# AiRyunn/BoT

Hardware: AMD Instinct MI355X
Metric: edges/sec full-batch GAT fwd+bwd on ogbn-arxiv; achieved HBM GB/s vs peak (higher is better)
Workload: dtype f32

## Files before the change

bot_amd/_C.py:

```python
from __future__ import annotations

import ctypes
import os
from ctypes import c_char_p, c_double, c_float, c_int32, c_int64, c_uint64, c_void_p

import torch

_HERE = os.path.dirname(os.path.abspath(__file__))
LIB_PATH = os.environ.get("BOT_AMD_LIB") or os.path.join(_HERE, "lib", "libbot_gnn.so")
ABI_VERSION = 19

if not os.path.exists(LIB_PATH):
    raise ImportError(
        f"{LIB_PATH} is missing: build the gfx950 kernels first "
        "(`make -C bot_amd/csrc` or `python -c 'import __graft_entry__ as g; g.build()'`). "
        "bot_amd has no CPU / PyTorch fallback."
    )
_lib = ctypes.CDLL(LIB_PATH)

_P = c_void_p
_SIGS = {
    "bot_abi_version": (ctypes.c_int, []),
    "bot_last_error": (c_char_p, []),
    "bot_last_kernel": (c_char_p, []),
# ... 897 lines not shown
    def fits(self, m, n, k) -> bool:
        return (m == self.n and n == self.F and self.F % 2 == 0 and self.x.stride(0) % 2 == 0 and self.x.data_ptr() % 8 == 0 and
                _lib.bot_gemm_halves3_nt_bn_rows(int(k)) == 256)

    def struct(self):
        return _BnBwdStats(self.x.data_ptr(), self.x.stride(0), self.mean.data_ptr(), self.invstd.data_ptr(), _ptr(self.weight), _ptr(self.bias),
                           int(self.relu), self.p, self.seed, _seed_off(self.p), self.part.data_ptr(), _ptr(self.pmax))

    def sums(self):
        sg = torch.empty(self.F, dtype=torch.float32, device=self.x.device)
        sgx = torch.empty(self.F, dtype=torch.float32, device=self.x.device)
        _check(_lib.bot_bn_act_bwd_reduce_partials_f32(self.part.data_ptr(), self.nblk, self.F, sg.data_ptr(), sgx.data_ptr(), _stream()),
               "bn_act_bwd_reduce_partials")
        return sg, sgx

    def finish(self, batch_stats, total_count, slots):
        assert self.pmax is not None
        _dev(slots)
        sg = torch.empty(self.F, dtype=torch.float32, device=self.x.device)
        sgx = torch.empty(self.F, dtype=torch.float32, device=self.x.device)
        _check(_lib.bot_bn_bwd_partials_finish_f32(self.part.data_ptr(), self.pmax.data_ptr(), self.nblk, self.F, sg.data_ptr(), sgx.data_ptr(),
                                                   int(bool(batch_stats)), float(total_count), _ptr(self.weight), self.invstd.data_ptr(), slots.data_ptr(),
                                                   _stream()), "bn_bwd_partials_finish")
        return sg, sgx

    def bound(self, sum_g, sum_gx, total_count, slots):
        assert self.pmax is not None
        _dev(slots)
        _check(_lib.bot_bn_bwd_bound_partials_f32(self.F, self.pmax.data_ptr(), self.nblk, _ptr(sum_g), _ptr(sum_gx), float(total_count), _ptr(self.weight),
                                                  self.invstd.data_ptr(), slots.data_ptr(), _stream()), "bn_bwd_bound_partials")
        return slots


def gemm_halves3_nt(a, b, scale_a, scale_b, piece_a, piece_b, k, out=None, mode=0, a2_off=None, scale_a2=None, k_split=0, b_frag=False, n=None, bn=None):
    _dev(a, b, scale_a, scale_b, scale_a2)
    m = a.shape[0]
    if n is None:
        assert not b_frag
        n = b.shape[0]
    if out is None:
        out = torch.empty((m, n), dtype=torch.float32, device=a.device)
    st = None
    if bn is not None:
        if not bn.fits(m, n, k):
            raise BotKernelError("gemm_halves3_nt: this product cannot carry the BatchNorm-backward by-product (BnBwdStats.fits)")
        st = bn.struct()
    _check(_timed("gemm_halves", (m, n, 3 * k, 1), lambda: _lib.bot_gemm_halves3_nt3_f32(
        m, n, k, scale_a.data_ptr(), _ptr(scale_a2), int(k_split), scale_b.data_ptr(), a.data_ptr(), _ld(a), 2 * piece_a if a2_off is None else a2_off,
        b.data_ptr(), _ld(b), piece_b, int(bool(b_frag)), out.data_ptr(), _ld(out), ctypes.addressof(st) if st is not None else None, int(mode), _stream())),
        "gemm_halves3_nt")
    return out


def halves_split_frag(x, scale, piece):
    _dev(x, scale)
    x = _mat(x, "x")
    n, F = x.shape
    assert piece % 64 == 0 and piece >= F
    out = torch.empty((2 * ((n + 15) // 16) * (piece // 32), 512), dtype=torch.float16, device=x.device)
    _check(_lib.bot_halves_split_frag_f16(x.data_ptr(), x.stride(0), n, F, _ptr(scale), out.data_ptr(), piece, _stream()), "halves_split_frag")
    return out


def _table(rows, width):
    flat = [int(v) for r in rows for v in r]
    assert len(flat) == width * len(rows)
    return (ctypes.c_int64 * len(flat))(*flat)


def gemm_halves3_nt_grouped(a, b, scale_a, scale_b, a2_off, b2_off, out, groups, k_seg, mode=0, col_scale=None, col_shift=None, relu=False, absmax=None,
                            stats=None):
    _dev(a, b, out, scale_a, scale_b, col_scale, col_shift, absmax)
    assert a.dtype == torch.float16 and b.dtype == torch.float16 and a.dim() == 2 and b.dim() == 2 and a.stride(1) == 1 and b.stride(1) == 1
    assert out.dtype == torch.float32 and out.stride(-1) == 1
    tab = _table(groups, 6)
    sp = sm = sv = None
    sF = 0
    if stats is not None:
        sp, sm, sv = stats
        _dev(sp, sm, sv)
        sF = sv.shape[1]
        tiles = (a.shape[0] + 255) // 256
        assert sp.shape == (tiles, 2, sF) and sm.shape == (tiles, 2, sF) and sv.shape == (tiles, sF)
        assert sp.is_contiguous() and sm.is_contiguous() and sv.is_contiguous()
        assert sp.dtype == sm.dtype == sv.dtype == torch.float32
    _check(_timed("gemm_halves", (a.shape[0], sum(int(g[1]) * 96 * int(g[4]) for g in groups), 1, 1), lambda: _lib.bot_gemm_halves3_nt_grouped2_f32(
        a.shape[0], b.shape[0], scale_a.data_ptr(), scale_b.data_ptr(), a.data_ptr(), _ld(a), a2_off, b.data_ptr(), _ld(b), b2_off, out.data_ptr(),
        int(out.stride(-2)), len(groups), tab, int(k_seg), _ptr(col_scale), _ptr(col_shift), int(bool(relu)), _ptr(absmax), _ptr(sp), _ptr(sm), _ptr(sv),
        int(sF), int(mode), _stream())), "gemm_halves3_nt_grouped")
    return out


def gemm_halves3_tn_grouped(x, d, scale_x, scale_d, x2_off, d2_off, out, tiles, mode=0):
    _dev(x, d, out, scale_x, scale_d)
    assert x.dtype == torch.float16 and d.dtype == torch.float16 and x.stride(1) == 1 and d.stride(1) == 1 and x.shape[0] == d.shape[0]
    assert out.dtype == torch.float32 and out.is_contiguous()
    n = x.shape[0]
    ws = torch.empty(int(_lib.bot_gemm_halves3_tn_grouped_workspace_floats(n, len(tiles))), dtype=torch.float32, device=x.device)
    tab = _table(tiles, 7)
    _check(_timed("gemm_halves", (n, sum(3 * int(t[1]) * int(t[3]) for t in tiles), 1, 1), lambda: _lib.bot_gemm_halves3_tn_grouped_f32(
        n, scale_x.data_ptr(), scale_d.data_ptr(), x.data_ptr(), _ld(x), x2_off, d.data_ptr(), _ld(d), d2_off, out.data_ptr(), len(tiles), tab,
        ws.data_ptr(), int(mode), _stream())), "gemm_halves3_tn_grouped")
    return out


def gemm_halves3_tn(x, d, scale_x, scale_d, piece_x, piece_d, k, p, mode=0, x2_off=None, d2_off=None, scale_d2=None, p_split=0):
    _dev(x, d, scale_x, scale_d, scale_d2)
    n = x.shape[0]
    out = torch.empty((k, p), dtype=torch.float32, device=x.device)
    ws = torch.empty(int(_lib.bot_gemm_halves3_tn_workspace_floats(n, piece_x, piece_d)), dtype=torch.float32, device=x.device)
    _check(_timed("gemm_halves", (k, p, 3 * n, 1), lambda: _lib.bot_gemm_halves3_tn2_f32(
        n, k, p, piece_x, piece_d, scale_x.data_ptr(), scale_d.data_ptr(), _ptr(scale_d2), int(p_split), x.data_ptr(), _ld(x),
        2 * piece_x if x2_off is None else x2_off, d.data_ptr(), _ld(d), 2 * piece_d if d2_off is None else d2_off,
        out.data_ptr(), _ld(out), ws.data_ptr(), int(mode), _stream())), "gemm_halves3_tn")
    return out


def _idx64(t, name):
    if t.dtype != torch.int64 or not t.is_contiguous() or t.dim() != 1:
        raise BotKernelError(f"{name} must be a contiguous 1-D int64 tensor (got {t.dtype}, stride {tuple(t.stride())})")


# ... 568 lines not shown
```

bot_amd/csrc/halves3.hip:

```cpp
#include <hip/hip_fp16.h>

#include <stdlib.h>
#include <string.h>

#include <algorithm>
#include <type_traits>
#include <utility>

#include "common.h"

namespace bot {
namespace {

constexpr int BK = 32;

typedef _Float16 half8 __attribute__((ext_vector_type(8)));
typedef float f32x4 __attribute__((ext_vector_type(4)));

struct H3Args {
    const _Float16* A;
    const _Float16* B;
    const float* scale_a;
    const float* scale_b;
    float* C;
// ... 652 lines not shown
    if constexpr (BNB) {
#pragma unroll
        for (int e = 0; e < 4; ++e) {
#pragma unroll
            for (int o = 8; o < 64; o <<= 1) {
                b_s[e] += __shfl_xor(b_s[e], o);
                b_q[e] += __shfl_xor(b_q[e], o);
                b_gm[e] = fmaxf(b_gm[e], __shfl_xor(b_gm[e], o));
                b_xm[e] = fmaxf(b_xm[e], __shfl_xor(b_xm[e], o));
            }
        }
        if (lane < 8) {
            const int64_t F = p.N;
            float* ps = p.bnb_part + ((int64_t)tm * 2) * F + c0 + col;
#pragma unroll
            for (int e = 0; e < 4; ++e)
                if (e < b_nv) ps[e] = b_s[e], ps[F + e] = b_q[e];
            if (p.bnb_pmax) {
                float* pm = p.bnb_pmax + ((int64_t)tm * 2) * F + c0 + col;
#pragma unroll
                for (int e = 0; e < 4; ++e)
                    if (e < b_nv) pm[e] = b_gm[e], pm[F + e] = b_xm[e];
            }
        }
    }
}

__global__ __launch_bounds__(512) void gemm_halves3_nt64_kernel(H3Args p) { gemm_halves3_nt64_body<false, false>(p, nullptr); }
__global__ __launch_bounds__(512) void gemm_halves3_nt64_frag_kernel(H3Args p) { gemm_halves3_nt64_body<false, true>(p, nullptr); }
__global__ __launch_bounds__(512) void gemm_halves3_nt64_grouped_kernel(H3Args p, H3Groups groups) { gemm_halves3_nt64_body<true, false>(p, &groups); }
__global__ __launch_bounds__(512) void gemm_halves3_nt64_bnb_kernel(H3Args p) { gemm_halves3_nt64_body<false, false, true>(p, nullptr); }
__global__ __launch_bounds__(512) void gemm_halves3_nt64_frag_bnb_kernel(H3Args p) { gemm_halves3_nt64_body<false, true, true>(p, nullptr); }

static bool nt64_wanted() {
    static const bool wanted = [] {
        const char* e = getenv("BOT_NT_KERNEL");
        return !(e && !strcmp(e, "128x64"));
    }();
    return wanted;
}

constexpr int TBK = 32;
constexpr int TT = 192;
constexpr int kTnSubA = TBK * 256, kTnSubB = TBK * 128;
constexpr int kTnPiece = kTnSubA + kTnSubB;
constexpr int kTnStage = 4 * kTnPiece;
constexpr int kTnStages = 3;

struct TnArgs3 {
    const _Float16* X;
    const _Float16* D;
    float* part;
    int64_t ldx, ldd;
    int N, K, P, KP, PP;
    int x2_off, d2_off;
    int tiles_k, tiles_p, splits, rows_per_split;
    int mode;
};


struct TnTile {
    int x_col0, d_col0, k_valid, p_valid;
    int64_t out_off, ldo;
    int transposed, pad;
};
constexpr int kMaxTnTiles = 16;
// ... 273 lines not shown
}

template <int BM, int BN, int WM, int WN, bool PIPE, bool ABLATE>
void launch_h3(H3Args p, int64_t m, int64_t n, hipStream_t st) {
    p.tiles_m = (int)((m + BM - 1) / BM), p.tiles_n = (int)((n + BN - 1) / BN);
    const int groups = (p.tiles_m + 7) / 8;
    hipLaunchKernelGGL((gemm_halves3_nt_kernel<BM, BN, WM, WN, PIPE, ABLATE>), dim3(groups * 8 * p.tiles_n), dim3(WM * WN * 64), 0, st, p);
}

}
}

extern "C" int bot_gemm_halves3_nt_f32(int64_t m, int64_t n, int64_t k, const float* scale_a, const float* scale_b, const uint16_t* A, int64_t lda,
                                       int64_t a2_off, const uint16_t* B, int64_t ldb, int64_t b2_off, float* C, int64_t ldc, int32_t mode,
                                       bot_stream_t stream) {
    return bot_gemm_halves3_nt2_f32(m, n, k, scale_a, nullptr, 0, scale_b, A, lda, a2_off, B, ldb, b2_off, 0, C, ldc, mode, stream);
}

extern "C" int bot_gemm_halves3_nt2_f32(int64_t m, int64_t n, int64_t k, const float* scale_a, const float* scale_a2, int64_t k_split, const float* scale_b,
                                        const uint16_t* A, int64_t lda, int64_t a2_off, const uint16_t* B, int64_t ldb, int64_t b2_off, int32_t b_layout,
                                        float* C, int64_t ldc, int32_t mode, bot_stream_t stream) {
    return bot_gemm_halves3_nt3_f32(m, n, k, scale_a, scale_a2, k_split, scale_b, A, lda, a2_off, B, ldb, b2_off, b_layout, C, ldc, nullptr, mode, stream);
}

extern "C" int32_t bot_gemm_halves3_nt_bn_rows(int64_t k) {
    using namespace bot;
    return (k > 0 && k % (2 * BK) == 0 && nt64_wanted()) ? 256 : 0;
}

extern "C" int bot_gemm_halves3_nt3_f32(int64_t m, int64_t n, int64_t k, const float* scale_a, const float* scale_a2, int64_t k_split, const float* scale_b,
                                        const uint16_t* A, int64_t lda, int64_t a2_off, const uint16_t* B, int64_t ldb, int64_t b2_off, int32_t b_layout,
                                        float* C, int64_t ldc, const bot_bn_bwd_stats_t* bn, int32_t mode, bot_stream_t stream) {
    using namespace bot;
    BOT_REQUIRE(bn == nullptr || (mode == 0 && bot_gemm_halves3_nt_bn_rows(k) == 256), -1,
                "gemm_halves3_nt3: the BatchNorm-backward by-product rides on the 256 x 32 form (mode 0, k a multiple of 64, BOT_NT_KERNEL not 128x64)");
    BOT_REQUIRE(bn == nullptr || (bn->x && bn->mean && bn->invstd && bn->part), -1, "gemm_halves3_nt3: bn->x, mean, invstd and part must be set");
    BOT_REQUIRE(bn == nullptr || (n % 2 == 0 && bn->ldx >= n && bn->ldx % 2 == 0 && aligned(bn->x, 8) && bn->p >= 0.f && bn->p < 1.f), -1,
                "gemm_halves3_nt3: the by-product needs an even n (= the BatchNorm width), 8-byte aligned x rows of pitch >= n and p in [0, 1)");
    BOT_REQUIRE(b_layout == 0 || (b_layout == 1 && mode == 0 && k % 64 == 0), -1,
                "gemm_halves3_nt2: b_layout 1 (fragment-major B, bot_halves_split_frag_f16 with piece = k) needs mode 0 and k a multiple of 64");
    BOT_REQUIRE(scale_a2 == nullptr || (k_split > 0 && k_split < k && k_split % BK == 0), -1,
                "gemm_halves3_nt2: the second scale starts at a column that is a positive multiple of %d below k (got %lld of %lld)", BK, (long long)k_split,
                (long long)k);
    BOT_REQUIRE(m > 0 && n > 0 && k > 0 && k % BK == 0, -1, "gemm_halves3_nt: m, n > 0 and k a positive multiple of %d (got %lld %lld %lld)", BK,
                (long long)m, (long long)n, (long long)k);
    BOT_REQUIRE(scale_a && scale_b && A && B && C, -1, "gemm_halves3_nt: null pointer");
    BOT_REQUIRE(aligned(A, 16) && aligned(B, 16) && lda % 8 == 0 && ldb % 8 == 0 && a2_off % 8 == 0 && b2_off % 8 == 0, -1,
                "gemm_halves3_nt: operands, row pitches and piece offsets must be 16-byte aligned");
    BOT_REQUIRE(a2_off + k <= lda && (b_layout == 1 || b2_off + k <= ldb) && ldc >= n && m < (1ll << 31) - 256 && n < (1ll << 31) - 256, -1, "gemm_halves3_nt: bad pitches");
    BOT_REQUIRE(b_layout == 0 || ((n + 15) / 16) * (k / 32) * 2048 < (1ll << 31), -1, "gemm_halves3_nt2: fragment-major B exceeds the 2 GiB a buffer descriptor spans");
    H3Args p;
    p.A = reinterpret_cast<const _Float16*>(A), p.B = reinterpret_cast<const _Float16*>(B), p.scale_a = scale_a, p.scale_b = scale_b, p.C = C;
    p.lda = lda, p.ldb = ldb, p.ldc = ldc, p.M = (int)m, p.N = (int)n, p.K = (int)k, p.a2_off = (int)a2_off, p.b2_off = (int)b2_off;
    p.tiles_m = p.tiles_n = 0;
    p.col_scale = p.col_shift = nullptr, p.relu = 0, p.absmax = nullptr;
    p.scale_a2 = scale_a2, p.k2 = scale_a2 ? (int)(k_split / BK) : -1;
    p.b_frag = b_layout;
    p.stats_part = p.stats_minmax = nullptr, p.stats_pivot = nullptr, p.stats_F = 0;
    p.bnb_x = nullptr, p.bnb_ldx = 0, p.bnb_mean = p.bnb_invstd = p.bnb_w = p.bnb_b = nullptr, p.bnb_relu = 0, p.bnb_p = 0.f, p.bnb_seed = 0;
    p.bnb_seed_offset = nullptr, p.bnb_part = p.bnb_pmax = nullptr;
    p.mode = mode;
    const bool force_128x64 = (mode & 1024) != 0;
    mode &= ~1024;
    p.mode = mode;
    if (bn) {
        p.bnb_x = bn->x, p.bnb_ldx = bn->ldx, p.bnb_mean = bn->mean, p.bnb_invstd = bn->invstd, p.bnb_w = bn->weight, p.bnb_b = bn->bias;
        p.bnb_relu = bn->relu, p.bnb_p = bn->p, p.bnb_seed = bn->seed, p.bnb_seed_offset = bn->seed_offset, p.bnb_part = bn->part, p.bnb_pmax = bn->pmax;
        p.tiles_m = (int)((m + 255) / 256), p.tiles_n = (int)((n + 255) / 256);
        set_kernel(b_layout ? "bot::gemm_halves3_nt64_frag_bnb_kernel" : "bot::gemm_halves3_nt64_bnb_kernel");
        if (b_layout) hipLaunchKernelGGL(gemm_halves3_nt64_frag_bnb_kernel, dim3(((p.tiles_m + 7) / 8) * 8 * p.tiles_n), dim3(512), 0, (hipStream_t)stream, p);
        else hipLaunchKernelGGL(gemm_halves3_nt64_bnb_kernel, dim3(((p.tiles_m + 7) / 8) * 8 * p.tiles_n), dim3(512), 0, (hipStream_t)stream, p);
    } else if (mode == 0 && !force_128x64 && nt64_wanted() && (k / BK) % 2 == 0) {
        p.tiles_m = (int)((m + 255) / 256), p.tiles_n = (int)((n + 255) / 256);
        set_kernel(b_layout ? "bot::gemm_halves3_nt64_frag_kernel" : "bot::gemm_halves3_nt64_kernel");
        if (b_layout) hipLaunchKernelGGL(gemm_halves3_nt64_frag_kernel, dim3(((p.tiles_m + 7) / 8) * 8 * p.tiles_n), dim3(512), 0, (hipStream_t)stream, p);
        else hipLaunchKernelGGL(gemm_halves3_nt64_kernel, dim3(((p.tiles_m + 7) / 8) * 8 * p.tiles_n), dim3(512), 0, (hipStream_t)stream, p);
    } else if (b_layout) {
        BOT_REQUIRE(false, -1, "gemm_halves3_nt2: a fragment-major B is read by the 256 x 32 form only (BOT_NT_KERNEL=128x64 / mode bit 1024 exclude it)");
    } else if (mode & 32) {
        set_kernel("bot::gemm_halves3_nt_kernel<256,256,2,4,plain>");
        launch_h3<256, 256, 2, 4, false, true>(p, m, n, (hipStream_t)stream);
    } else if (mode) {
        set_kernel("bot::gemm_halves3_nt_kernel<256,256,2,4,pipelined,ablate>");
        launch_h3<256, 256, 2, 4, true, true>(p, m, n, (hipStream_t)stream);
    } else {
        set_kernel("bot::gemm_halves3_nt_kernel<256,256,2,4,pipelined>");
        launch_h3<256, 256, 2, 4, true, false>(p, m, n, (hipStream_t)stream);
    }
    return hip_status("gemm_halves3_nt");
}

extern "C" int bot_gemm_halves3_nt_grouped_f32(int64_t m, int64_t b_rows, const float* scale_a, const float* scale_b, const uint16_t* A, int64_t lda,
                                               int64_t a2_off, const uint16_t* B, int64_t ldb, int64_t b2_off, float* C, int64_t ldc, int32_t n_groups,
                                               const int64_t* groups, int32_t k_seg, const float* col_scale, const float* col_shift, int32_t relu,
                                               uint32_t* absmax_slots, int32_t mode, bot_stream_t stream) {
    return bot_gemm_halves3_nt_grouped2_f32(m, b_rows, scale_a, scale_b, A, lda, a2_off, B, ldb, b2_off, C, ldc, n_groups, groups, k_seg, col_scale, col_shift,
                                            relu, absmax_slots, nullptr, nullptr, nullptr, 0, mode, stream);
}
// ... 7 lines not shown
    BOT_REQUIRE((stats_part == nullptr) == (stats_minmax == nullptr) && (stats_part == nullptr) == (stats_pivot == nullptr) && (stats_part == nullptr || stats_F >= 1), -1,
                "gemm_halves3_nt_grouped2: stats_part, stats_minmax and stats_pivot go together (stats_F = their row width)");
    BOT_REQUIRE(m > 0 && b_rows > 0 && n_groups >= 1 && n_groups <= kMaxGroups && k_seg >= 0, -1, "gemm_halves3_nt_grouped: m, b_rows > 0, 1 .. %d groups (got %lld %lld %d)",
                kMaxGroups, (long long)m, (long long)b_rows, n_groups);
    BOT_REQUIRE(scale_a && scale_b && A && B && C && groups, -1, "gemm_halves3_nt_grouped: null pointer");
    BOT_REQUIRE(aligned(A, 16) && aligned(B, 16) && lda % 8 == 0 && ldb % 8 == 0 && a2_off % 8 == 0 && b2_off % 8 == 0, -1,
                "gemm_halves3_nt_grouped: operands, row pitches and piece offsets must be 16-byte aligned");
    BOT_REQUIRE(m < (1ll << 31) - 256 && b_rows < (1ll << 31) - 256 && 256 * lda * 2 < (1ll << 31) && 256 * ldb * 2 < (1ll << 31), -1, "gemm_halves3_nt_grouped: bad sizes");
    H3Args p;
    p.A = reinterpret_cast<const _Float16*>(A), p.B = reinterpret_cast<const _Float16*>(B), p.scale_a = scale_a, p.scale_b = scale_b, p.C = C;
    p.lda = lda, p.ldb = ldb, p.ldc = ldc, p.M = (int)m, p.N = (int)b_rows, p.K = 0, p.a2_off = (int)a2_off, p.b2_off = (int)b2_off;
    p.mode = 0;
    p.scale_a2 = nullptr, p.k2 = -1, p.b_frag = 0;
    p.stats_part = stats_part, p.stats_minmax = stats_minmax, p.stats_pivot = stats_pivot, p.stats_F = stats_F;
    p.col_scale = col_scale, p.col_shift = col_shift, p.relu = relu, p.absmax = absmax_slots;
    H3Groups g;
    g.k_seg = k_seg;
    for (int i = 0; i < n_groups; ++i) {
        const int64_t* d = groups + 6 * i;
        const int64_t k_steps = d[4], a_hi = std::max(k_seg > 0 ? d[2] + 32 * std::min<int64_t>(k_seg, k_steps) : 0, k_steps > k_seg ? d[3] + 32 * k_steps : 0);
        BOT_REQUIRE(d[0] >= 0 && d[0] < b_rows && d[1] >= 1 && d[1] <= 256 && k_steps >= 1 && d[2] >= 0 && d[3] >= 0 && d[2] % 8 == 0 && d[3] % 8 == 0 && d[5] >= 0, -1,
                    "gemm_halves3_nt_grouped: group %d: b_row0=%lld n_valid=%lld a_col0=%lld a_col1=%lld k_steps=%lld c_off=%lld", i, (long long)d[0],
                    (long long)d[1], (long long)d[2], (long long)d[3], (long long)d[4], (long long)d[5]);
        BOT_REQUIRE(a_hi + a2_off <= lda && 32 * k_steps + b2_off <= ldb && 32 * k_steps <= b2_off, -1,
                    "gemm_halves3_nt_grouped: group %d reads past a row (A columns to %lld + %lld of %lld, B columns to %lld + %lld of %lld)", i, (long long)a_hi,
                    (long long)a2_off, (long long)lda, (long long)(32 * k_steps), (long long)b2_off, (long long)ldb);
        g.g[i] = H3Group{(int)d[0], (int)d[1], (int)d[2] * 2, (int)d[3] * 2, (int)k_steps, 0, d[5]};
    }
    p.tiles_m = (int)((m + 255) / 256), p.tiles_n = n_groups;
    bool even = k_seg % 2 == 0;
    for (int i = 0; i < n_groups; ++i) even = even && g.g[i].k_steps % 2 == 0;
    BOT_REQUIRE(stats_part == nullptr || (!(mode & 1024) && even && nt64_wanted()), -1,
                "gemm_halves3_nt_grouped2: the statistics by-product exists in the 256 x 32 form only (even k-step counts, BOT_NT_KERNEL != 128x64)");
    if (!(mode & 1024) && even && nt64_wanted()) {
        set_kernel("bot::gemm_halves3_nt64_grouped_kernel");
        hipLaunchKernelGGL(gemm_halves3_nt64_grouped_kernel, dim3(((p.tiles_m + 7) / 8) * 8 * n_groups), dim3(512), 0, (hipStream_t)stream, p, g);
        return hip_status("gemm_halves3_nt_grouped");
    }
    set_kernel("bot::gemm_halves3_nt_grouped_kernel<256,256,2,4,pipelined>");
    hipLaunchKernelGGL((gemm_halves3_nt_grouped_kernel<256, 256, 2, 4, true>), dim3(((p.tiles_m + 7) / 8) * 8 * n_groups), dim3(512), 0, (hipStream_t)stream, p, g);
    return hip_status("gemm_halves3_nt_grouped");
}

namespace bot {
namespace {
int tn_splits(int64_t n_rows, int tiles) {
    const int64_t by_rows = n_rows / 4096;
    if (by_rows < 8) return (int)std::max<int64_t>(1, by_rows);
    int best_q = 1;
    double best = 0.0;
    for (int q = 1; q <= 8 && 8 * q <= by_rows; ++q) {
        const int wg = q * tiles, rounds = (wg + 31) / 32;
        const double eff = (double)wg / (32.0 * rounds);
        if (eff > best + 1e-9) best = eff, best_q = q;
    }
    return 8 * best_q;
}
}
}

namespace bot {
namespace {
int tn_grouped_splits(int64_t n_rows, int n_tiles) {
    const int per_xcd = std::max(1, 32 / n_tiles);
    return (int)std::max<int64_t>(1, std::min<int64_t>(8 * per_xcd, n_rows / 1024));
}
// ... 87 lines not shown
```

bot_amd/nn/fused.py:

```python
from __future__ import annotations

import os
from types import SimpleNamespace

import torch
import torch.nn as nn
import torch.nn.functional as F

from .. import _C, gemm, halo, side
from ..graph import take_rows
from ..ops import bn_epilogue_forward, bn_epilogue_sums, new_dropout_seed, stats_partials_for


ABSMAX_BYPRODUCT = os.environ.get("BOT_ABSMAX_BYPRODUCT", "1") != "0"
SKIP_Y = os.environ.get("BOT_SKIP_Y", "1") != "0"
HANDLES = 0
SKINNY = os.environ.get("BOT_SKINNY", "1") != "0"
FORCE = False
CALLS = 0
AGG_CALLS = 0
L0_CALLS = 0


def can_fuse(conv, norm, activation, graph, training, stack_residual) -> bool:
# ... 389 lines not shown
            return dWk if kp else dWk.t().contiguous()
        dW = side.run(wgrad, xh, buf, s1, s2) if (side.usable(buf) and xh.piece * piece >= side.MIN_OUT) else wgrad()
    return (dh, dW, d_bn_w if ctx.needs_input_grad[2] else None, d_bn_b if ctx.needs_input_grad[3] else None,
            None, None, None, None, None, None, None, None, None, None, None, None, None)


def cat_weight_aggfirst(conv):
    H, D = conv._num_heads, conv._out_feats
    W = conv.fc.weight
    Wh = W.view(H, D, -1)
    rows = [conv.res_fc.weight] if conv.res_fc is not None else []
    rows.append((Wh * conv.attn_l.view(H, D, 1)).sum(1))
    if conv.attn_r is not None:
        rows.append((Wh * conv.attn_r.view(H, D, 1)).sum(1))
    used = sum(r.shape[0] for r in rows)
    pad = (-used) % 128
    if pad:
        rows.append(W.new_zeros(pad, W.shape[1]))
    return torch.cat(rows)


WEIGHT_KP = True


def _kp(w):
    return w.t().contiguous() if WEIGHT_KP else w


AGG_FIRST = True


L0_HALVES = os.environ.get("BOT_L0_HALVES", "1") != "0"
L0_DIRECT = os.environ.get("BOT_L0_DIRECT", "1") != "0"
_L0_TABLES = {}
_L0_DH = {}


def _l0_dh(device, N, H, D, DP):
    key = (str(device), N, H, D, DP)
    buf = _L0_DH.get(key)
    if buf is None:
        buf = torch.zeros((N, 2 * H * DP), dtype=torch.float16, device=device)
        if not (buf.is_cuda and torch.cuda.is_current_stream_capturing()):
            _L0_DH[key] = buf
    return buf


def _l0_tables(H, D, Fin, P2, kp, N):
    key = (H, D, Fin, P2, kp, N)
    if key not in _L0_TABLES:
        FP = (Fin + 63) // 64 * 64
        DP = (D + 63) // 64 * 64
        HD = H * D
        fwd = [(h * D, D, 0, h * FP, 2 * FP // 32, h * D) for h in range(H)]
        dz = [(h * Fin, Fin, 0, h * DP, DP // 32, h * N * Fin) for h in range(H)]
        tn = []
        for h in range(H):
            for j in range((D + 127) // 128):
                pv = min(128, D - 128 * j)
                col = h * D + 128 * j
                tn.append((FP * (1 + h), Fin, h * DP + 128 * j, pv, col * Fin, Fin, 1))
                if kp:
                    tn.append((0, Fin, h * DP + 128 * j, pv, HD * Fin + col, P2, 0))
                else:
                    tn.append((0, Fin, h * DP + 128 * j, pv, HD * Fin + col * Fin, Fin, 1))
        _L0_TABLES[key] = (FP, DP, fwd, dz, tn)
# ... 118 lines not shown
        h, W, Wr, z, table, el, er, a, a_d = s.h, s.W, s.Wr, s.z, s.table, s.el, s.er, s.a, s.a_d
        dy = dy.contiguous()
        d_bn_w = d_bn_b = None
        l0h, kp = ctx.l0h, ctx.kp
        N, Fin, HD, P2 = h.shape[0], h.shape[1], H * D, Wr.shape[1 if kp else 0]
        Nd = g.number_of_dst_nodes()
        dout2 = torch.empty((N, P2), dtype=h.dtype, device=h.device)
        dx = dout2[:Nd, :HD] if has_res else torch.empty((Nd, HD), dtype=h.dtype, device=h.device)
        if has_res and Nd < N:
            dout2[Nd:, :HD].zero_()
        direct = l0h and L0_DIRECT and epi is not None and D % 2 == 0
        slots = _C.absmax_slots(dy.device) if l0h and (ABSMAX_BYPRODUCT or direct) and epi is not None else None
        Dh = dscale = None
        if epi is None:
            dx.copy_(dy)
        else:
            (sg, sgx), (d_bn_b, d_bn_w) = bn_epilogue_sums(epi, dy, s.x, s.mean, s.invstd, s.bn_w, s.bn_b, True, epi.bn_training and epi.sync,
                                                           slots if direct else None)
            if direct:
                DP = (D + 63) // 64 * 64
                dscale = _C.halves_scale_from_slots(slots)
                Dh = _C.bn_act_bwd_apply_halves(dy, s.x, s.mean, s.invstd, s.bn_w, s.bn_b, True, epi.drop_p, epi.seed, sg, sgx, epi.total,
                                                dscale, _l0_dh(dy.device, Nd, H, D, DP), D, DP)
            else:
                _C.bn_act_bwd_apply(dy, s.x, s.mean, s.invstd, s.bn_w, s.bn_b, True, epi.drop_p, epi.seed, sg, sgx, epi.total, out=dx, absmax=slots)
        Wh = W.view(H, D, Fin)
        dz = torch.empty((H, Nd, Fin), dtype=h.dtype, device=h.device)
        dW3 = torch.empty((H, D, Fin), dtype=h.dtype, device=h.device) if ctx.needs_input_grad[1] and not l0h else None
        if l0h:
            FP, DP, _, g_dz, t_tn = _l0_tables(H, D, Fin, P2, kp, Nd)
            if Dh is None:
                dscale = _C.halves_scale_from_slots(slots) if slots is not None else _C.halves_scale(dx)
                Dh = _C.halves_split_heads(dx, dscale, H, D, DP)
            Wt = gemm.split(Wh.transpose(1, 2).reshape(H * Fin, D), 1)
            _C.gemm_halves3_nt_grouped(Dh, Wt.buf, dscale, Wt.scale, H * DP, Wt.piece, dz[0], g_dz, 0)
            flat = torch.empty(HD * Fin + P2 * Fin, dtype=h.dtype, device=h.device)

            def wgrad():
                _C.gemm_halves3_tn_grouped(z, Dh, s.xscale, dscale, (1 + H) * FP, H * DP, flat, t_tn)
                return flat
            if side.usable(flat):
                side.run(wgrad, z, Dh, s.xscale, dscale, flat)
            else:
                wgrad()
        elif ctx.skinny and D <= 256:
            _C.skinny_gemm(dx, Wh, b_is_kn=True, out=dz, batch=H, strides=(D, D * Fin, Nd * Fin), m=Nd, n=Fin, k=D)
        if ctx.skinny and dW3 is not None:
            _C.tn_gemm(dx, z, out=dW3, batch=H, strides=(D, Nd * Fin, 0), n=Nd, kx=D, ky=Fin)
        for i in range(H if not l0h else 0):
            dxi = dx[:, i * D:(i + 1) * D]
            if not (ctx.skinny and D <= 256):
                torch.mm(dxi, Wh[i], out=dz[i])
            if dW3 is not None and not ctx.skinny:
                torch.mm(dxi.t(), z[i], out=dW3[i])
        dW = dW3.view(HD, Fin) if dW3 is not None else None
        halo = g.halo is not None
        c = HD if has_res else 0
        need_dh = ctx.needs_input_grad[0]
        if not need_dh:
            xsrc = table[:, :Fin] if halo else h
            da = _C.sddmm_dot_bcast(g.csc, xsrc, dz)
            dh_g = None
        elif halo:
            dext = torch.empty_like(table)
            _, da = _C.spmm_dot_bcast(g.csr, dz, a_d, g.csr2csc, table[:, :Fin], out=dext[:, :Fin])
        else:
            dh_g, da = _C.spmm_dot_bcast(g.csr, dz, a_d, g.csr2csc, h)
        d_el, der = _attn_backward(ctx, da, el, er, a)
        if halo and not need_dh:
            dsm = d_el.new_zeros((d_el.shape[0], (H + 3) // 4 * 4))
            dsm[:, :H] = d_el
            d_el = _extend_backward(g, dsm, N)[:, :H]
        elif halo:
            _score_columns(dext, Fin, d_el)
            own = _extend_backward(g, dext, N)
            dh_g, d_el = own[:, :Fin], own[:, Fin:Fin + H]
        _score_columns(dout2, c, d_el, der)
# ... 281 lines not shown
```

Measured before the change: 239.4 million.

## Add 256x128 short-reduction NT GEMM form and fork weight-grad stream earlier

Adds a new NT GEMM kernel family with a 256x128 block tile (each wave owning 256x16), two-stage LDS double buffering and launch bounds allowing four blocks. The dispatcher picks it automatically for short reductions (at most 24 k-steps) with poorly filled 256-wide tiles. It is meant to cut wasted columns and raise occupancy on skinny GEMMs. Separately, the layer-0 backward now launches the side-stream weight-gradient GEMM before the dz grouped GEMM, so the two can overlap. Both paths are on by default and add new kernel variants and mode bits that can be forced or disabled.

```diff
diff --git a/bot_amd/_C.py b/bot_amd/_C.py
--- a/bot_amd/_C.py
+++ b/bot_amd/_C.py
@@ -953,6 +953,17 @@
         return slots
 
 
+NT_128x64, NT_SHORT, NT_NO_SHORT = 1024, 2048, 4096
+NT_FORM = 0
+NT_FORM_COUNTS = None
+
+
+def _nt_count():
+    if NT_FORM_COUNTS is not None:
+        name = _lib.bot_last_kernel().decode()
+        NT_FORM_COUNTS[name] = NT_FORM_COUNTS.get(name, 0) + 1
+
+
 def gemm_halves3_nt(a, b, scale_a, scale_b, piece_a, piece_b, k, out=None, mode=0, a2_off=None, scale_a2=None, k_split=0, b_frag=False, n=None, bn=None):
     _dev(a, b, scale_a, scale_b, scale_a2)
     m = a.shape[0]
@@ -968,8 +979,9 @@
         st = bn.struct()
     _check(_timed("gemm_halves", (m, n, 3 * k, 1), lambda: _lib.bot_gemm_halves3_nt3_f32(
         m, n, k, scale_a.data_ptr(), _ptr(scale_a2), int(k_split), scale_b.data_ptr(), a.data_ptr(), _ld(a), 2 * piece_a if a2_off is None else a2_off,
-        b.data_ptr(), _ld(b), piece_b, int(bool(b_frag)), out.data_ptr(), _ld(out), ctypes.addressof(st) if st is not None else None, int(mode), _stream())),
-        "gemm_halves3_nt")
+        b.data_ptr(), _ld(b), piece_b, int(bool(b_frag)), out.data_ptr(), _ld(out), ctypes.addressof(st) if st is not None else None, int(mode) or NT_FORM,
+        _stream())), "gemm_halves3_nt")
+    _nt_count()
     return out
 
 
@@ -1008,7 +1020,8 @@
     _check(_timed("gemm_halves", (a.shape[0], sum(int(g[1]) * 96 * int(g[4]) for g in groups), 1, 1), lambda: _lib.bot_gemm_halves3_nt_grouped2_f32(
         a.shape[0], b.shape[0], scale_a.data_ptr(), scale_b.data_ptr(), a.data_ptr(), _ld(a), a2_off, b.data_ptr(), _ld(b), b2_off, out.data_ptr(),
         int(out.stride(-2)), len(groups), tab, int(k_seg), _ptr(col_scale), _ptr(col_shift), int(bool(relu)), _ptr(absmax), _ptr(sp), _ptr(sm), _ptr(sv),
-        int(sF), int(mode), _stream())), "gemm_halves3_nt_grouped")
+        int(sF), int(mode) or NT_FORM, _stream())), "gemm_halves3_nt_grouped")
+    _nt_count()
     return out
 
 
diff --git a/bot_amd/csrc/halves3.hip b/bot_amd/csrc/halves3.hip
--- a/bot_amd/csrc/halves3.hip
+++ b/bot_amd/csrc/halves3.hip
@@ -708,6 +708,365 @@
 __global__ __launch_bounds__(512) void gemm_halves3_nt64_bnb_kernel(H3Args p) { gemm_halves3_nt64_body<false, false, true>(p, nullptr); }
 __global__ __launch_bounds__(512) void gemm_halves3_nt64_frag_bnb_kernel(H3Args p) { gemm_halves3_nt64_body<false, true, true>(p, nullptr); }
 
+template <bool GROUPED, bool BFRAG, bool BNB = false>
+__device__ __forceinline__ void gemm_halves3_nts_body(const H3Args& p, const H3Groups* groups) {
+    static_assert(!(GROUPED && BNB) && !(GROUPED && BFRAG), "grouped launches: row-major B, no BatchNorm-backward by-product");
+    constexpr int BM = 256, BN = 128, kWaves = 8, MT = BM / 16;
+    constexpr int kABytes = BM * BK * 2;
+    constexpr int kStageBytes = 2 * kABytes, kStages = 2;
+    constexpr int GA = BM / 16 / kWaves;
+    static_assert(GA == 2 && BN == kWaves * 16, "wave tile 256 x 16");
+    __shared__ __attribute__((aligned(1024))) unsigned char lds[kStages * kStageBytes];
+    const int tid = threadIdx.x, lane = tid & 63, w = __builtin_amdgcn_readfirstlane(tid >> 6);
+    const int b = blockIdx.x, xcd = b & 7, j = b >> 3;
+    const int tm = (j / p.tiles_n) * 8 + xcd, tn = j % p.tiles_n;
+    if (tm >= p.tiles_m) return;
+    const int m0 = tm * BM;
+    int n0 = tn * BN, n_valid = p.N - n0, T = p.K / BK, a_off0 = 0, a_off1 = 0, k_seg = 0;
+    int64_t c0 = n0;
+    if constexpr (GROUPED) {
+        const H3Group& G = groups->g[tn >> 1];
+        const int half = (tn & 1) * BN;
+        n0 = G.b_row0 + half, n_valid = G.n_valid - half, T = G.k_steps, a_off0 = G.a_off0, a_off1 = G.a_off1, c0 = G.c_off + half, k_seg = groups->k_seg;
+        if (n_valid <= 0) return;
+    }
+    const bool active = w * 16 < n_valid;
+    const float alpha = (p.scale_a2 ? p.scale_a2[1] : p.scale_a[1]) * p.scale_b[1];
+
+    const _Float16* tileA = p.A + (int64_t)m0 * p.lda;
+    const int nb = min(n0, p.N - 1);
+    const _Float16* tileB = p.B + (int64_t)nb * p.ldb;
+    const int lr = lane >> 2, cq = (lane & 3) ^ ((-(lane >> 4)) & 3);
+    uint32_t offA[GA];
+#pragma unroll
+    for (int h = 0; h < GA; ++h) offA[h] = ((uint32_t)(min(m0 + (w + kWaves * h) * 16 + lr, p.M - 1) - m0) * (uint32_t)p.lda + cq * 8) * 2;
+    const int a2b = p.a2_off * 2;
+    auto issue_a = [&](int i, int stage, int kt) {
+        const int q = i / GA, h = i % GA;
+        dma16(tileA, lds + stage * kStageBytes + q * kABytes + (w + kWaves * h) * 1024, offA[h],
+              (GROUPED ? kt * (BK * 2) + (kt < k_seg ? a_off0 : a_off1) : kt * (BK * 2)) + q * a2b);
+    };
+    const int Tk = p.K / BK;
+    uint32_t offB;
+    int tileoff = 0;
+    if constexpr (BFRAG) {
+        offB = lane * 16;
+        tileoff = min((n0 + w * 16) >> 4, ((p.N + 15) >> 4) - 1) * Tk * 1024;
+    } else {
+        offB = ((uint32_t)(min(n0 + w * 16 + (lane & 15), p.N - 1) - nb) * (uint32_t)p.ldb) * 2 + (lane >> 4) * 16;
+    }
+    const int b2 = BFRAG ? ((p.N + 15) >> 4) * Tk * 1024 : p.b2_off * 2;
+    const _Float16* baseB = BFRAG ? p.B : tileB;
+    auto load_b = [&](half8& x1, half8& x2, int kt) {
+        const int so = BFRAG ? tileoff + kt * 1024 : kt * (BK * 2);
+        x1 = load16(baseB, offB, so);
+        x2 = load16(baseB, offB, so + b2);
+    };
+    const int frow = lane & 15;
+    const int a_off = frow * 64 + (((lane >> 4) ^ ((-(frow >> 2)) & 3)) * 16);
+
+    f32x4 acc[MT];
+#pragma unroll
+    for (int mt = 0; mt < MT; ++mt) acc[mt] = f32x4{0.f, 0.f, 0.f, 0.f};
+    const _Float16 sh = (_Float16)(1.0f / kHalvesShift);
+
+    half8 x1 = {}, x2 = {}, y1 = {}, y2 = {};
+#pragma unroll
+    for (int i = 0; i < 2 * GA; ++i) issue_a(i, 0, 0);
+    if (active) load_b(x1, x2, 0);
+    asm volatile("s_waitcnt vmcnt(0)" ::: "memory");
+    __builtin_amdgcn_s_barrier();
+    asm volatile("" : "+v"(x1), "+v"(x2));
+    auto kstep = [&](int t, auto more_tag) {
+        constexpr bool more = decltype(more_tag)::value;
+        const unsigned char* st = lds + (t & 1) * kStageBytes;
+        if (active) {
+            if constexpr (more) load_b(y1, y2, t + 1);
+            if (t == p.k2) {
+                const float r = p.scale_a2[0] * p.scale_a[1];
+#pragma unroll
+                for (int mt = 0; mt < MT; ++mt) acc[mt] = acc[mt] * r;
+            }
+            const half8 bs = x1 * sh;
+            half8 a1 = *reinterpret_cast<const half8*>(st + a_off);
+            half8 a2 = *reinterpret_cast<const half8*>(st + a_off + kABytes);
+#pragma unroll
+            for (int mt = 0; mt < MT; ++mt) {
+                half8 an1 = a1, an2 = a2;
+                if (mt + 1 < MT) {
+                    an1 = *reinterpret_cast<const half8*>(st + a_off + (mt + 1) * 1024);
+                    an2 = *reinterpret_cast<const half8*>(st + a_off + kABytes + (mt + 1) * 1024);
+                }
+                if constexpr (more) {
+                    if (mt < 2 * GA) issue_a(mt, (t + 1) & 1, t + 1);
+                }
+                acc[mt] = __builtin_amdgcn_mfma_f32_16x16x32_f16(x1, a1, acc[mt], 0, 0, 0);
+                acc[mt] = __builtin_amdgcn_mfma_f32_16x16x32_f16(x2, a1, acc[mt], 0, 0, 0);
+                acc[mt] = __builtin_amdgcn_mfma_f32_16x16x32_f16(bs, a2, acc[mt], 0, 0, 0);
+                a1 = an1, a2 = an2;
+            }
+        } else {
+            if constexpr (more) {
+#pragma unroll
+                for (int i = 0; i < 2 * GA; ++i) issue_a(i, (t + 1) & 1, t + 1);
+            }
+        }
+        asm volatile("s_waitcnt vmcnt(0) lgkmcnt(0)" ::: "memory");
+        __builtin_amdgcn_s_barrier();
+        asm volatile("" ::: "memory");
+        if constexpr (more) x1 = y1, x2 = y2;
+    };
+    int t = 0;
+    for (; t + 1 < T; ++t) kstep(t, std::true_type{});
+    kstep(t, std::false_type{});
+    if (!active) return;
+
+    float* const Cb = p.C + c0;
+    const bool vec_ok = (p.ldc % 4 == 0) && ((reinterpret_cast<uintptr_t>(Cb) & 15) == 0);
+    const bool vec2_ok = (p.ldc % 2 == 0) && ((reinterpret_cast<uintptr_t>(Cb) & 7) == 0);
+    constexpr int P = 16 + 4;
+    static_assert(32 * P * 4 <= kStages * kStageBytes / kWaves, "staging slab does not fit the wave's share of the LDS");
+    float* stg = reinterpret_cast<float*>(lds + w * (kStages * kStageBytes / kWaves));
+    const int q4 = (lane >> 4) * 4, l15 = lane & 15, l3 = lane & 3, rl = lane >> 2;
+    const int col = w * 16 + l3 * 4;
+    float cs[4] = {1.f, 1.f, 1.f, 1.f}, ch[4] = {0.f, 0.f, 0.f, 0.f};
+    const bool affine = GROUPED && (p.col_scale != nullptr || p.col_shift != nullptr);
+    const bool relu = GROUPED && p.relu;
+    const bool want_amax = GROUPED && p.absmax != nullptr;
+    if (affine) {
+#pragma unroll
+        for (int e = 0; e < 4; ++e)
+            if (col + e < n_valid) {
+                if (p.col_scale) cs[e] = p.col_scale[c0 + col + e];
+                if (p.col_shift) ch[e] = p.col_shift[c0 + col + e];
+            }
+    }
+    float amax = 0.f;
+    const bool stats = GROUPED && p.stats_part != nullptr;
+    float st_s[4] = {0.f, 0.f, 0.f, 0.f}, st_q[4] = {0.f, 0.f, 0.f, 0.f}, st_mn[4], st_mx[4], piv[4] = {0.f, 0.f, 0.f, 0.f};
+#pragma unroll
+    for (int e = 0; e < 4; ++e) st_mn[e] = INFINITY, st_mx[e] = -INFINITY;
+    float b_s[4] = {0.f, 0.f, 0.f, 0.f}, b_q[4] = {0.f, 0.f, 0.f, 0.f}, b_gm[4] = {0.f, 0.f, 0.f, 0.f}, b_xm[4] = {0.f, 0.f, 0.f, 0.f};
+    float* const bcst = stg + 32 * P + l3 * 4;
+    int b_nv = 0;
+    bool b_wide = false;
+    uint64_t b_seed = 0;
+    int64_t b_nquad = 0;
+    float b_keep = 1.f;
+    if constexpr (BNB) {
+        b_nv = max(0, min(4, n_valid - col));
+#pragma unroll
+        for (int e = 0; e < 4; ++e)
+            if (lane < 4) {
+                const bool in = e < b_nv;
+                bcst[e] = in ? p.bnb_mean[c0 + col + e] : 0.f, bcst[16 + e] = in ? p.bnb_invstd[c0 + col + e] : 0.f;
+                bcst[32 + e] = in && p.bnb_w ? p.bnb_w[c0 + col + e] : 1.f, bcst[48 + e] = in && p.bnb_b ? p.bnb_b[c0 + col + e] : 0.f;
+            }
+        b_wide = (p.bnb_ldx % 4 == 0) && ((reinterpret_cast<uintptr_t>(p.bnb_x) & 15) == 0);
+        b_seed = p.bnb_seed_offset ? p.bnb_seed + p.bnb_seed_offset[0] * 0x9E3779B97F4A7C15ull : p.bnb_seed;
+        b_nquad = (p.N + 3) / 4;
+        b_keep = p.bnb_p > 0.f ? 1.f / (1.f - p.bnb_p) : 1.f;
+    }
+    f32x4 b_ring[2][2];
+    auto load_x = [&](auto pass_c) __attribute__((always_inline)) {
+        constexpr int pass = decltype(pass_c)::value;
+        if constexpr (BNB && pass < MT / 2) {
+#pragma unroll
+            for (int i = 0; i < 2; ++i) {
+                const int row = m0 + pass * 32 + i * 16 + rl;
+                f32x4& q = b_ring[pass % 2][i];
+                q = f32x4{0.f, 0.f, 0.f, 0.f};
+                if (row < p.M && b_nv > 0) {
+                    const float* xp = p.bnb_x + (int64_t)row * p.bnb_ldx + c0 + col;
+                    if (b_wide && b_nv == 4) {
+                        q = *reinterpret_cast<const f32x4*>(xp);
+                    } else {
+                        const float2 lo = *reinterpret_cast<const float2*>(xp);
+                        q[0] = lo.x, q[1] = lo.y;
+                        if (b_nv == 4) {
+                            const float2 hi = *reinterpret_cast<const float2*>(xp + 2);
+                            q[2] = hi.x, q[3] = hi.y;
+                        }
+                    }
+                }
+            }
+        }
+    };
+    load_x(std::integral_constant<int, 0>{});
+    auto do_pass = [&](auto pass_c) __attribute__((always_inline)) {
+        constexpr int pass = decltype(pass_c)::value;
+        load_x(std::integral_constant<int, pass + 1>{});
+#pragma unroll
+        for (int mm = 0; mm < 2; ++mm) {
+            const f32x4 v = acc[pass * 2 + mm] * alpha;
+            *reinterpret_cast<f32x4*>(stg + (mm * 16 + l15) * P + q4) = v;
+        }
+#pragma unroll
+        for (int i = 0; i < 2; ++i) {
+            const int r = i * 16 + rl;
+            f32x4 v = *reinterpret_cast<const f32x4*>(stg + r * P + l3 * 4);
+            const int row = m0 + pass * 32 + r;
+            if (affine || relu) {
+#pragma unroll
+                for (int e = 0; e < 4; ++e) {
+                    v[e] = fmaf(v[e], cs[e], ch[e]);
+                    if (relu) v[e] = fmaxf(v[e], 0.f);
+                }
+            }
+            if constexpr (GROUPED) {
+                if constexpr (pass == 0) {
+                    if (stats && i == 0) {
+#pragma unroll
+                        for (int e = 0; e < 4; ++e) piv[e] = __shfl(v[e], l3);
+                    }
+                }
+                if (stats) {
+                    float vo[4];
+#pragma unroll
+                    for (int e = 0; e < 4; ++e) vo[e] = __shfl_xor(v[e], 32);
+#pragma unroll
+                    for (int u = 0; u < 2; ++u) {
+                        if (row + 8 * u < p.M) {
+#pragma unroll
+                            for (int e = 0; e < 4; ++e) {
+                                const float x = u ? vo[e] : v[e];
+                                const float d = x - piv[e];
+                                st_s[e] += d;
+                                st_q[e] = fmaf(d, d, st_q[e]);
+                                st_mn[e] = fminf(st_mn[e], x), st_mx[e] = fmaxf(st_mx[e], x);
+                            }
+                        }
+                    }
+                }
+            }
+            if constexpr (BNB) {
+                float gg[4] = {0.f, 0.f, 0.f, 0.f}, xh[4] = {0.f, 0.f, 0.f, 0.f};
+                if (row < p.M && b_nv > 0) {
+                    float f[4] = {1.f, 1.f, 1.f, 1.f};
+                    if (p.bnb_p > 0.f) {
+                        uint32_t wd[4];
+                        Philox::gen(b_seed, (uint64_t)((int64_t)row * b_nquad + ((c0 + col) >> 2)), wd);
+#pragma unroll
+                        for (int e = 0; e < 4; ++e) f[e] = ((wd[e] >> 8) * (1.0f / 16777216.0f)) >= p.bnb_p ? b_keep : 0.f;
+                    }
+                    const f32x4 b_mu = *reinterpret_cast<const f32x4*>(bcst), b_is = *reinterpret_cast<const f32x4*>(bcst + 16);
+                    const f32x4 b_sc = *reinterpret_cast<const f32x4*>(bcst + 32), b_sh = *reinterpret_cast<const f32x4*>(bcst + 48);
+#pragma unroll
+                    for (int e = 0; e < 4; ++e) {
+                        xh[e] = (b_ring[pass % 2][i][e] - b_mu[e]) * b_is[e];
+                        gg[e] = v[e] * f[e];
+                        if (p.bnb_relu && !(fmaf(xh[e], b_sc[e], b_sh[e]) > 0.f)) gg[e] = 0.f;
+                    }
+                }
+                float go[4], xo[4];
+#pragma unroll
+                for (int e = 0; e < 4; ++e) go[e] = __shfl_xor(gg[e], 32), xo[e] = __shfl_xor(xh[e], 32);
+#pragma unroll
+                for (int u = 0; u < 2; ++u) {
+                    if (row + 8 * u < p.M && b_nv > 0) {
+#pragma unroll
+                        for (int e = 0; e < 4; ++e) {
+                            const float g1 = u ? go[e] : gg[e], x1h = u ? xo[e] : xh[e];
+                            if (e < b_nv) {
+                                b_s[e] += g1;
+                                b_q[e] = fmaf(g1, x1h, b_q[e]);
+                                b_gm[e] = fmaxf(b_gm[e], fabsf(g1)), b_xm[e] = fmaxf(b_xm[e], fabsf(x1h));
+                            }
+                        }
+                    }
+                }
+            }
+            if (want_amax && row < p.M) {
+#pragma unroll
+                for (int e = 0; e < 4; ++e)
+                    if (col + e < n_valid) amax = fmaxf(amax, fabsf(v[e]));
+            }
+            if (row < p.M) {
+                float* c = Cb + (int64_t)row * p.ldc + col;
+                if (vec_ok && col + 3 < n_valid) {
+                    *reinterpret_cast<float4*>(c) = make_float4(v[0], v[1], v[2], v[3]);
+                } else if (vec2_ok && col + 3 < n_valid) {
+                    *reinterpret_cast<float2*>(c) = make_float2(v[0], v[1]);
+                    *reinterpret_cast<float2*>(c + 2) = make_float2(v[2], v[3]);
+                } else {
+#pragma unroll
+                    for (int e = 0; e < 4; ++e)
+                        if (col + e < n_valid) c[e] = v[e];
+                }
+            }
+        }
+    };
+    static_for<MT / 2>(do_pass);
+    if constexpr (GROUPED) {
+        if (want_amax) {
+            const float wm = wave_absmax(amax);
+            if (lane == 0) {
+                const uint32_t bits = __float_as_uint(wm);
+                uint32_t* sl = p.absmax + (((((tm >> 3) * (p.tiles_n >> 1) + (tn >> 1)) << 3) + xcd) & (kAbsmaxSlots - 1));
+                if (bits > __hip_atomic_load(sl, __ATOMIC_RELAXED, __HIP_MEMORY_SCOPE_AGENT)) atomicMax(sl, bits);
+            }
+        }
+        if (stats) {
+#pragma unroll
+            for (int e = 0; e < 4; ++e) {
+#pragma unroll
+                for (int o = 4; o < 32; o <<= 1) {
+                    st_s[e] += __shfl_xor(st_s[e], o);
+                    st_q[e] += __shfl_xor(st_q[e], o);
+                    st_mn[e] = fminf(st_mn[e], __shfl_xor(st_mn[e], o));
+                    st_mx[e] = fmaxf(st_mx[e], __shfl_xor(st_mx[e], o));
+                }
+            }
+            if (lane < 4) {
+                const int64_t F = p.stats_F;
+                float* ps = p.stats_part + ((int64_t)tm * 2) * F + c0 + col;
+                float* pm = p.stats_minmax + ((int64_t)tm * 2) * F + c0 + col;
+                float* pp = p.stats_pivot + (int64_t)tm * F + c0 + col;
+#pragma unroll
+                for (int e = 0; e < 4; ++e)
+                    if (col + e < n_valid) ps[e] = st_s[e], ps[F + e] = st_q[e], pm[e] = st_mn[e], pm[F + e] = st_mx[e], pp[e] = piv[e];
+            }
+        }
+    }
+    if constexpr (BNB) {
+#pragma unroll
+        for (int e = 0; e < 4; ++e) {
+#pragma unroll
+            for (int o = 4; o < 32; o <<= 1) {
+                b_s[e] += __shfl_xor(b_s[e], o);
+                b_q[e] += __shfl_xor(b_q[e], o);
+                b_gm[e] = fmaxf(b_gm[e], __shfl_xor(b_gm[e], o));
+                b_xm[e] = fmaxf(b_xm[e], __shfl_xor(b_xm[e], o));
+            }
+        }
+        if (lane < 4) {
+            const int64_t F = p.N;
+            float* ps = p.bnb_part + ((int64_t)tm * 2) * F + c0 + col;
+#pragma unroll
+            for (int e = 0; e < 4; ++e)
+                if (e < b_nv) ps[e] = b_s[e], ps[F + e] = b_q[e];
+            if (p.bnb_pmax) {
+                float* pm = p.bnb_pmax + ((int64_t)tm * 2) * F + c0 + col;
+#pragma unroll
+                for (int e = 0; e < 4; ++e)
+                    if (e < b_nv) pm[e] = b_gm[e], pm[F + e] = b_xm[e];
+            }
+        }
+    }
+}
+
+__global__ __launch_bounds__(512, 4) void gemm_halves3_nts_kernel(H3Args p) { gemm_halves3_nts_body<false, false>(p, nullptr); }
+__global__ __launch_bounds__(512, 4) void gemm_halves3_nts_frag_kernel(H3Args p) { gemm_halves3_nts_body<false, true>(p, nullptr); }
+__global__ __launch_bounds__(512, 4) void gemm_halves3_nts_grouped_kernel(H3Args p, H3Groups groups) { gemm_halves3_nts_body<true, false>(p, &groups); }
+__global__ __launch_bounds__(512, 4) void gemm_halves3_nts_bnb_kernel(H3Args p) { gemm_halves3_nts_body<false, false, true>(p, nullptr); }
+__global__ __launch_bounds__(512, 4) void gemm_halves3_nts_frag_bnb_kernel(H3Args p) { gemm_halves3_nts_body<false, true, true>(p, nullptr); }
+
+constexpr int kModeShort = 2048, kModeNoShort = 4096;
+
+static bool nt_short_wanted(int64_t k_steps, int64_t used16, int64_t total16, bool byproduct) {
+    return !byproduct && k_steps <= 24 && (k_steps <= 4 || 4 * used16 <= 3 * total16);
+}
+
 static bool nt64_wanted() {
     static const bool wanted = [] {
         const char* e = getenv("BOT_NT_KERNEL");
@@ -1047,12 +1406,12 @@
                                         const uint16_t* A, int64_t lda, int64_t a2_off, const uint16_t* B, int64_t ldb, int64_t b2_off, int32_t b_layout,
                                         float* C, int64_t ldc, const bot_bn_bwd_stats_t* bn, int32_t mode, bot_stream_t stream) {
     using namespace bot;
-    BOT_REQUIRE(bn == nullptr || (mode == 0 && bot_gemm_halves3_nt_bn_rows(k) == 256), -1,
+    BOT_REQUIRE(bn == nullptr || ((mode & ~(bot::kModeShort | bot::kModeNoShort)) == 0 && bot_gemm_halves3_nt_bn_rows(k) == 256), -1,
                 "gemm_halves3_nt3: the BatchNorm-backward by-product rides on the 256 x 32 form (mode 0, k a multiple of 64, BOT_NT_KERNEL not 128x64)");
     BOT_REQUIRE(bn == nullptr || (bn->x && bn->mean && bn->invstd && bn->part), -1, "gemm_halves3_nt3: bn->x, mean, invstd and part must be set");
     BOT_REQUIRE(bn == nullptr || (n % 2 == 0 && bn->ldx >= n && bn->ldx % 2 == 0 && aligned(bn->x, 8) && bn->p >= 0.f && bn->p < 1.f), -1,
                 "gemm_halves3_nt3: the by-product needs an even n (= the BatchNorm width), 8-byte aligned x rows of pitch >= n and p in [0, 1)");
-    BOT_REQUIRE(b_layout == 0 || (b_layout == 1 && mode == 0 && k % 64 == 0), -1,
+    BOT_REQUIRE(b_layout == 0 || (b_layout == 1 && (mode & ~(bot::kModeShort | bot::kModeNoShort)) == 0 && k % 64 == 0), -1,
                 "gemm_halves3_nt2: b_layout 1 (fragment-major B, bot_halves_split_frag_f16 with piece = k) needs mode 0 and k a multiple of 64");
     BOT_REQUIRE(scale_a2 == nullptr || (k_split > 0 && k_split < k && k_split % BK == 0), -1,
                 "gemm_halves3_nt2: the second scale starts at a column that is a positive multiple of %d below k (got %lld of %lld)", BK, (long long)k_split,
@@ -1076,9 +1435,23 @@
     p.bnb_seed_offset = nullptr, p.bnb_part = p.bnb_pmax = nullptr;
     p.mode = mode;
     const bool force_128x64 = (mode & 1024) != 0;
-    mode &= ~1024;
+    const bool force_short = (mode & kModeShort) != 0, no_short = (mode & kModeNoShort) != 0;
+    mode &= ~(1024 | kModeShort | kModeNoShort);
     p.mode = mode;
-    if (bn) {
+    BOT_REQUIRE(!(force_short && (force_128x64 || no_short || mode != 0)), -1, "gemm_halves3_nt: mode bit %d (the short-reduction form) goes with no other bit", kModeShort);
+    if (force_short || (mode == 0 && !force_128x64 && !no_short && nt64_wanted() && nt_short_wanted(k / BK, (n + 15) / 16, 16 * ((n + 255) / 256), bn != nullptr))) {
+        p.tiles_m = (int)((m + 255) / 256), p.tiles_n = (int)((n + 127) / 128);
+        if (bn) {
+            p.bnb_x = bn->x, p.bnb_ldx = bn->ldx, p.bnb_mean = bn->mean, p.bnb_invstd = bn->invstd, p.bnb_w = bn->weight, p.bnb_b = bn->bias;
+            p.bnb_relu = bn->relu, p.bnb_p = bn->p, p.bnb_seed = bn->seed, p.bnb_seed_offset = bn->seed_offset, p.bnb_part = bn->part, p.bnb_pmax = bn->pmax;
+        }
+        const dim3 grid(((p.tiles_m + 7) / 8) * 8 * p.tiles_n);
+        set_kernel("bot::gemm_halves3_nts%s%s_kernel", b_layout ? "_frag" : "", bn ? "_bnb" : "");
+        if (bn && b_layout) hipLaunchKernelGGL(gemm_halves3_nts_frag_bnb_kernel, grid, dim3(512), 0, (hipStream_t)stream, p);
+        else if (bn) hipLaunchKernelGGL(gemm_halves3_nts_bnb_kernel, grid, dim3(512), 0, (hipStream_t)stream, p);
+        else if (b_layout) hipLaunchKernelGGL(gemm_halves3_nts_frag_kernel, grid, dim3(512), 0, (hipStream_t)stream, p);
+        else hipLaunchKernelGGL(gemm_halves3_nts_kernel, grid, dim3(512), 0, (hipStream_t)stream, p);
+    } else if (bn) {
         p.bnb_x = bn->x, p.bnb_ldx = bn->ldx, p.bnb_mean = bn->mean, p.bnb_invstd = bn->invstd, p.bnb_w = bn->weight, p.bnb_b = bn->bias;
         p.bnb_relu = bn->relu, p.bnb_p = bn->p, p.bnb_seed = bn->seed, p.bnb_seed_offset = bn->seed_offset, p.bnb_part = bn->part, p.bnb_pmax = bn->pmax;
         p.tiles_m = (int)((m + 255) / 256), p.tiles_n = (int)((n + 255) / 256);
@@ -1152,6 +1525,16 @@
     for (int i = 0; i < n_groups; ++i) even = even && g.g[i].k_steps % 2 == 0;
     BOT_REQUIRE(stats_part == nullptr || (!(mode & 1024) && even && nt64_wanted()), -1,
                 "gemm_halves3_nt_grouped2: the statistics by-product exists in the 256 x 32 form only (even k-step counts, BOT_NT_KERNEL != 128x64)");
+    int max_steps = 0, used16 = 0;
+    for (int i = 0; i < n_groups; ++i) max_steps = std::max(max_steps, g.g[i].k_steps), used16 += (g.g[i].n_valid + 15) / 16;
+    const bool force_short = (mode & kModeShort) != 0;
+    BOT_REQUIRE(!(force_short && (mode & (1024 | kModeNoShort))), -1, "gemm_halves3_nt_grouped: mode bit %d (the short-reduction form) goes with no other bit", kModeShort);
+    if (force_short || (!(mode & (1024 | kModeNoShort)) && nt64_wanted() && nt_short_wanted(max_steps, used16, 16 * n_groups, stats_part != nullptr))) {
+        p.tiles_n = 2 * n_groups;
+        set_kernel("bot::gemm_halves3_nts_grouped_kernel");
+        hipLaunchKernelGGL(gemm_halves3_nts_grouped_kernel, dim3(((p.tiles_m + 7) / 8) * 8 * p.tiles_n), dim3(512), 0, (hipStream_t)stream, p, g);
+        return hip_status("gemm_halves3_nt_grouped");
+    }
     if (!(mode & 1024) && even && nt64_wanted()) {
         set_kernel("bot::gemm_halves3_nt64_grouped_kernel");
         hipLaunchKernelGGL(gemm_halves3_nt64_grouped_kernel, dim3(((p.tiles_m + 7) / 8) * 8 * n_groups), dim3(512), 0, (hipStream_t)stream, p, g);
diff --git a/bot_amd/nn/fused.py b/bot_amd/nn/fused.py
--- a/bot_amd/nn/fused.py
+++ b/bot_amd/nn/fused.py
@@ -445,6 +445,7 @@
 
 L0_HALVES = os.environ.get("BOT_L0_HALVES", "1") != "0"
 L0_DIRECT = os.environ.get("BOT_L0_DIRECT", "1") != "0"
+L0_FORK_EARLY = os.environ.get("BOT_L0_FORK_EARLY", "1") != "0"
 _L0_TABLES = {}
 _L0_DH = {}
 
@@ -629,17 +630,23 @@
             if Dh is None:
                 dscale = _C.halves_scale_from_slots(slots) if slots is not None else _C.halves_scale(dx)
                 Dh = _C.halves_split_heads(dx, dscale, H, D, DP)
-            Wt = gemm.split(Wh.transpose(1, 2).reshape(H * Fin, D), 1)
-            _C.gemm_halves3_nt_grouped(Dh, Wt.buf, dscale, Wt.scale, H * DP, Wt.piece, dz[0], g_dz, 0)
             flat = torch.empty(HD * Fin + P2 * Fin, dtype=h.dtype, device=h.device)
 
             def wgrad():
                 _C.gemm_halves3_tn_grouped(z, Dh, s.xscale, dscale, (1 + H) * FP, H * DP, flat, t_tn)
                 return flat
-            if side.usable(flat):
-                side.run(wgrad, z, Dh, s.xscale, dscale, flat)
-            else:
-                wgrad()
+
+            def fork():
+                if side.usable(flat):
+                    side.run(wgrad, z, Dh, s.xscale, dscale, flat)
+                else:
+                    wgrad()
+            if L0_FORK_EARLY:
+                fork()
+            Wt = gemm.split(Wh.transpose(1, 2).reshape(H * Fin, D), 1)
+            _C.gemm_halves3_nt_grouped(Dh, Wt.buf, dscale, Wt.scale, H * DP, Wt.piece, dz[0], g_dz, 0)
+            if not L0_FORK_EARLY:
+                fork()
         elif ctx.skinny and D <= 256:
             _C.skinny_gemm(dx, Wh, b_is_kn=True, out=dz, batch=H, strides=(D, D * Fin, Nd * Fin), m=Nd, n=Fin, k=D)
         if ctx.skinny and dW3 is not None:
```

After: 242.7 million (median of 6 runs). +1.4%, better.
